# 412428728/ksched

Hardware: AMD Instinct MI355X
Metric: MCMF solve latency (ms) + arcs/s at 100k tasks x 10k machines, 1/2/4/8 GPUs (higher is better)
Workload: dtype int64; 1 GPU; config3: Quincy-shaped cell graph T=100000 M=10000 R=250 J=1000 (n=121252, m=531250), step = full device re-solve + device task->PU extraction (Solve() -> TaskMapping), one graph per GPU; tasks=100000, machines=10000, racks=250, jobs=1000, seed=3, n=121252, m=531250, parallelism=independent graphs x1

## Files before the change

include/ksmcmf.h:

```cpp
#ifndef KSMCMF_H
#define KSMCMF_H

#include <stddef.h>
#include <stdint.h>

#ifdef __cplusplus
extern "C" {
#endif

#define KSMCMF_ABI_VERSION 5

#define KS_OK            0
#define KS_E_INVALID    (-1)
#define KS_E_INFEASIBLE (-2)
#define KS_E_DEVICE     (-3)
#define KS_E_VERIFY     (-4)
#define KS_E_RANGE      (-5)

#define KS_NODE_OTHER    0
#define KS_NODE_TASK     1
#define KS_NODE_PU       2
#define KS_NODE_SINK     3
#define KS_NODE_MACHINE  4
#define KS_NODE_INTERMEDIATE 5
// ... 82 lines not shown
    uint64_t sweep_launches;
    double   ms_sweep_kernels;
    uint64_t gu_launches;
    double   ms_gu_kernels;
    int32_t  warm_started;
    int32_t  rebuilt;
    int32_t  recoveries;
    int32_t  solver;
    uint64_t fs_launches;
    double   ms_fs_kernels;
    uint64_t fwd_updates;
    int32_t  cells;
    int32_t  compact;
    double   ms_cell_kernel;
    uint64_t cell_ticks_max;
    uint64_t cell_ticks_sum;
    uint64_t fs_arc_scans;
    uint64_t cell_fallbacks;
    uint64_t cycles_cancelled;
    uint64_t fb_resets;
    uint64_t cycles_rejected;
    uint64_t gu_leaf_scans;
    int32_t  cells_run;
    int32_t  reserved4;
    uint64_t reserved3[1];
} ks_result;

typedef struct ks_store_stats {
    int64_t  live_arcs;
    int64_t  inserted;
    int64_t  updated;
    int64_t  killed;
    int64_t  superseded;
    int64_t  rebuilds;
    int64_t  residual_slots;
    int64_t  reserved[4];
} ks_store_stats;

typedef struct ks_flow {
    uint64_t src, dst;
    int64_t  flow;
} ks_flow;

int         ks_abi_version(void);
void        ks_default_opts(ks_opts* opts);
ks_ctx*     ks_create(int device, const ks_opts* opts);
void        ks_destroy(ks_ctx* ctx);
const char* ks_last_error(ks_ctx* ctx);
// ... 299 lines not shown
```

ksched_amd/csrc/ks_engine.hip:

```cpp
#include <hip/hip_runtime.h>

#include <algorithm>
#include <chrono>
#include <cstdio>
#include <cstdlib>
#include <cstring>
#include <vector>

#include "ks_engine_impl.h"
#include "ks_len.h"

namespace ks {
namespace {

__device__ __forceinline__ void seg_of(const long long* nd, int x, int& b0, int& b1) {
    const unsigned long long w = (unsigned long long)nd[ni(x) + ND_SEG];
    b0 = (int)(unsigned)(w & 0xffffffffULL);
    b1 = (int)(unsigned)(w >> 32);
}

__device__ __forceinline__ long long atom_add_ret(long long* p, long long v) {
    return __hip_atomic_fetch_add(p, v, __ATOMIC_RELAXED, __HIP_MEMORY_SCOPE_AGENT);
}
__device__ __forceinline__ long long atom_exch(long long* p, long long v) {
// ... 1074 lines not shown
                                         int& out, int& scans, int& lscan) {
    const int lig = lane_id() & (G - 1);
    long long dv = INF64;
    if (v >= 0) dv = atom_load(&g.dist[ni(v)]);
    const bool act = v >= 0 && (PR || dv < INF64);
    long long pv = 0;
    int b0 = 0, en = 0;
    if (act) {
        pv = g.p0[ni(v)];
        seg_of(g.p0, v, b0, en);
    }
    const int iters = G < 64 ? 1 : (en - b0 + 63) / 64;
    for (int it = 0; it < iters; ++it) {
        const int a = b0 + it * G + lig;
        if (a < en) {
            relax_in<PR, CP>(g, nf, Q, v, a, dkey<PR>(dv), pv, er, B, hub_min, out, lscan);
            scans++;
        }
    }
}

template <int PR, bool CP>
__global__ __launch_bounds__(BLK) void k_bf_round(DG g, int seq, int dense_arg) {
    const unsigned long long t_entry = PR == 2 ? __builtin_amdgcn_s_memrealtime() : 0;
    const int dense = __builtin_amdgcn_readfirstlane(dense_arg >= 0 ? dense_arg : (seq == g.ctl->bf_seq0 ? 1 : 0));
    __shared__ long long hub_min[HUB_LDS];
    __shared__ QEnt bfq[BF_DEPTH][BFQ_CAP];
    __shared__ int bfq_n[BF_DEPTH];
    if (blockIdx.x == 0) {
        for (int h = threadIdx.x; h < g.nheavy; h += BLK) g.bf[(seq + 2) % 3].hub[h] = 0;
        if (threadIdx.x == 0) g.ctl->bfa[(seq + 2) % 3] = 0;
    }
    const Front F = g.bf[seq % 3], N = g.bf[(seq + 1) % 3];
    if (threadIdx.x < HUB_LDS) hub_min[threadIdx.x] = INF64;
    if (threadIdx.x < BF_DEPTH) bfq_n[threadIdx.x] = 0;
    const int qcap = g.expand < 2 ? 0 : (g.expand == 2 ? BFQ_CAP : 2);
    const int qlo = qcap ? g.obeg[2] : 0, qhi = qcap ? g.obeg[CCLS] : 0;
    const BfQ Q{bfq[0], &bfq_n[0], qcap, qlo, qhi};
    __syncthreads();
    int done = 0, any = 0;
    auto ctl_words = [&]() {
        done = g.ctl->bf_done;
        any = g.ctl->bfa[seq % 3];
    };
    auto ctl_uniform = [&]() {
        done = __builtin_amdgcn_readfirstlane(done);
        any = __builtin_amdgcn_readfirstlane(any);
// ... 85 lines not shown
            const int qn = min(bfq_n[l], qcap);
            const BfQ Qn{bfq[l + 1 < BF_DEPTH ? l + 1 : 0], &bfq_n[l + 1 < BF_DEPTH ? l + 1 : 0],
                         l + 1 < BF_DEPTH ? qcap : 0, l + 1 < BF_DEPTH ? qlo : 0, l + 1 < BF_DEPTH ? qhi : 0};
            bf_drain<PR, CP>(g, N, bfq[l], qn, Qn, er, B, hub_min, out, scans, lscan);
            __syncthreads();
        }
    }
    if (threadIdx.x < HUB_LDS && (int)threadIdx.x < g.nheavy) {
        const long long val = hub_min[threadIdx.x];
        if (val < INF64) {
            long long* dx = &g.dist[ni(g.hub_base + threadIdx.x)];
            if (dless<PR>(val, atom_load(dx)) && dless<PR>(val, atom_min_ret(dx, val))) {
                N.hub[threadIdx.x] = 1;
                out = 1;
            }
        }
    }
    if (__any(out) && lane_id() == 0) g.ctl->bfa[(seq + 1) % 3] = 1;
    if (blockIdx.x == 0 && threadIdx.x == 0) {
        if (PR == 2 && g.ctl->t_srch) {
            g.ctl->srch_ticks += t_entry - g.ctl->t_srch;
            g.ctl->t_srch = 0;
        }
        if (!done && (dense || any)) {
            atomicAdd(g.ctr + C_BFROUND, 1ULL);
            g.ctl->bf_count += 1;
        } else if (!done) {
            g.ctl->bf_done = 1;
        }
    }
    if (!PR && g.bound && blockIdx.x == 0 && threadIdx.x < WAVE && !done && (dense || any)) {
        const int nb = g.ctl->n_bx;
        if (nb > 0 && nb <= BX_CAP) {
            long long d = 0;
            if ((int)threadIdx.x < nb) d = atom_load(&g.dist[ni(g.bx[threadIdx.x])]);
            d = wave_max(d);
            if (threadIdx.x == 0 && d < INF64)
                __hip_atomic_fetch_min(&g.ctl->bf_bound, d, __ATOMIC_RELAXED, __HIP_MEMORY_SCOPE_AGENT);
        }
    }
    scans = wave_sum(scans);
    lscan = wave_sum(lscan);
    if (lane_id() == 0 && (scans | lscan)) {
        const int sh = ((blockIdx.x * WPB) + (threadIdx.x >> 6)) & (CTR_SHARDS - 1);
        if (scans) atomicAdd(g.ctr + sh * NCTR + C_GUSCAN, (unsigned long long)scans);
        if (lscan) atomicAdd(g.ctr + sh * NCTR + C_GULEAF, (unsigned long long)lscan);
// ... 4 lines not shown
    for (long long i = blockIdx.x * (long long)BLK + threadIdx.x; i < g.hub_base; i += (long long)gridDim.x * BLK) {
        fs[0].flag[i] = 0;
        fs[1].flag[i] = 0;
        fs[2].flag[i] = 0;
    }
    if (blockIdx.x == 0)
        for (int h = threadIdx.x; h < g.nheavy; h += BLK) fs[0].hub[h] = fs[1].hub[h] = fs[2].hub[h] = 0;
}

__device__ __forceinline__ void bx_append(const DG& g, bool on, int v) {
    const unsigned long long m = __ballot(on);
    if (!m) return;
    int base = 0;
    if (lane_id() == 0) base = atomicAdd(&g.ctl->n_bx, (int)__popcll(m));
    base = __shfl(base, 0);
    if (on) {
        const int idx = base + (int)__popcll(m & ((1ULL << lane_id()) - 1));
        if (idx < BX_CAP) g.bx[idx] = v;
    }
}

__global__ void k_gu_init(DG g, int seq0, int list) {
    if (g.ctl->gu_pending) return;
    clear_fronts(g, g.bf);
    const Front F0 = g.bf[seq0 % 3];
    if (blockIdx.x == 0 && threadIdx.x == 0) {
        __hip_atomic_store(&g.ctl->bf_bound, INF64, __ATOMIC_RELAXED, __HIP_MEMORY_SCOPE_AGENT);
        g.ctl->gu_B = INF64;
        g.ctl->bf_done = 0;
        g.ctl->gu_L = 0;
        g.ctl->gu_X = -1;
        g.ctl->bf_r0 = g.ctl->bf_count;
        g.ctl->bf_seq0 = seq0;
        g.ctl->n_exc = 0;
        g.ctl->u_exc = 0;
        g.ctl->aug_reached = 0;
        g.ctl->aug_short = 0;
        for (int k = 0; k < 3; ++k) g.ctl->bfa[k] = k == seq0 % 3 ? 1 : 0;
    }
    for (long long v0 = blockIdx.x * (long long)BLK; v0 < g.hub_base; v0 += (long long)gridDim.x * BLK) {
        const long long v = v0 + threadIdx.x;
        long long e = 0;
        if (v < g.hub_base) {
            e = atom_load(&g.excess[v]);
            g.dist[ni(v)] = e < 0 ? 0 : INF64;
            if (e < 0) F0.flag[v] = 1;
// ... 5 lines not shown
            const int h = h0 + threadIdx.x;
            long long e = 0;
            if (h < g.nheavy) {
                drain_inbox(g, h);
                e = atom_load(&g.excess[g.hub_base + h]);
                g.dist[ni(g.hub_base + h)] = e < 0 ? 0 : INF64;
                if (e < 0) F0.hub[h] = 1;
            }
            if (list) bx_append(g, e > 0, g.hub_base + h);
        }
}

__global__ void k_pr_init(DG g, int seq0, int from_p) {
    clear_fronts(g, g.bf);
    if (blockIdx.x == 0 && threadIdx.x == 0) {
        g.ctl->bf_done = 0;
        g.ctl->bf_seq0 = seq0;
        for (int k = 0; k < 3; ++k) g.ctl->bfa[k] = 0;
    }
    for (long long v = blockIdx.x * (long long)BLK + threadIdx.x; v < g.n; v += (long long)gridDim.x * BLK)
        g.dist[ni(v)] = from_p == 2 ? ((PK_BIAS << PK_NB) | PK_NONE) : from_p ? g.p0[ni(v)] : 0;
}

__global__ void k_cycle_end(DG g, Ctl* host, int fwd) {
    static_assert(sizeof(Ctl) % 4 == 0, "Ctl is copied as words");
    const unsigned long long t = __builtin_amdgcn_s_memrealtime();
    if (threadIdx.x == 0) {
        if (!fwd) g.ctl->gu_pending = g.ctl->bf_done ? 0 : 1;
        g.ctl->t_end = t;
    }
    __syncthreads();
    const int* src = reinterpret_cast<const int*>(g.ctl);
    int* dst = reinterpret_cast<int*>(host);
    for (int i = threadIdx.x; i < (int)(sizeof(Ctl) / 4); i += blockDim.x)
        __hip_atomic_store(&dst[i], src[i], __ATOMIC_RELAXED, __HIP_MEMORY_SCOPE_SYSTEM);
    __syncthreads();
    if (threadIdx.x == 0) {
        if (!fwd) {
            g.ctl->n_exc = 0;
            g.ctl->u_exc = 0;
        }
        g.ctl->fs_moved_cyc = 0;
    }
    __threadfence_system();
}

constexpr int SET_FWD = 1;
constexpr int SET_CYC = 2;
__global__ void k_set_eps(DG g, long long eps, double inv, int flags) {
    g.ctl->eps = eps;
    g.ctl->inv = inv;
    g.ctl->lim = (1LL << 60) / eps;
// ... 3 lines not shown
        g.ctl->fs_completed = 0;
    }
    if (flags & SET_CYC) {
        g.ctl->cyc_done = 0;
        g.ctl->cyc_rej = 0;
    }
}

__global__ void k_prc_snap(DG g, Ctl* host) {
    const unsigned long long t = __builtin_amdgcn_s_memrealtime();
    if (threadIdx.x == 0 && g.ctl->t_srch) {
        g.ctl->srch_ticks += t - g.ctl->t_srch;
        g.ctl->t_srch = 0;
    }
    __syncthreads();
    const int* src = reinterpret_cast<const int*>(g.ctl);
    int* dst = reinterpret_cast<int*>(host);
    for (int i = threadIdx.x; i < (int)(sizeof(Ctl) / 4); i += blockDim.x)
        __hip_atomic_store(&dst[i], src[i], __ATOMIC_RELAXED, __HIP_MEMORY_SCOPE_SYSTEM);
    __threadfence_system();
}

__global__ void k_gu_max(DG g) {
    __shared__ long long sh[WPB];
    clear_fronts(g, g.sf);
    if (blockIdx.x == 0) {
        for (int k = threadIdx.x; k < MAXB; k += BLK) g.ctl->sweep_act[k] = 0;
        for (int h = threadIdx.x; h < g.nheavy; h += BLK) {
            g.aug_req[h] = 0;
        }
        if (threadIdx.x == 0) {
            g.ctl->apply_act = 0;
            g.ctl->n_xl2 = 0;
        }
    }
    if (!g.ctl->bf_done) return;
    if (g.bound && blockIdx.x == 0 && threadIdx.x < WAVE) {
        const int nb = g.ctl->n_bx;
        if (nb > 0 && nb <= BX_CAP) {
            long long d = 0;
            if ((int)threadIdx.x < nb) d = atom_load(&g.dist[ni(g.bx[threadIdx.x])]);
            d = wave_max(d);
            if (threadIdx.x == 0) g.ctl->gu_B = d;
        }
        if (threadIdx.x == 0) g.ctl->n_bx = 0;
    }
    long long mx = 0;
    long long mxx = -1;
    for (long long v = blockIdx.x * (long long)BLK + threadIdx.x; v < g.n; v += (long long)gridDim.x * BLK) {
        const long long d = atom_load(&g.dist[ni(v)]);
        if (d < INF64) mx = max(mx, d);
        if (d < INF64 && atom_load(&g.excess[v]) > 0) mxx = max(mxx, d);
    }
    mx = wave_max(mx);
    const int w = threadIdx.x >> 6;
    if (lane_id() == 0) sh[w] = mx;
// ... 1017 lines not shown
int Engine::device() const { return p_->device; }

int Engine::init(int device, const ks_opts& opts, std::string& err) {
    EngineImpl& s = *p_;
    s.device = device;
    s.opts = opts;
    int ndev = 0;
    KS_CHECK(hipGetDeviceCount(&ndev));
    if (device < 0 || device >= ndev) {
        err = "device index out of range";
        return KS_E_DEVICE;
    }
    KS_CHECK(hipSetDevice(device));
    KS_CHECK(hipStreamCreateWithFlags(&s.stream, hipStreamNonBlocking));
    {
        int v = 0;
        if (hipDeviceGetAttribute(&v, hipDeviceAttributeSharedMemPerBlockOptin, device) != hipSuccess || v <= 0)
            KS_CHECK(hipDeviceGetAttribute(&v, hipDeviceAttributeMaxSharedMemoryPerBlock, device));
        s.lds_limit = (size_t)std::max(v, 0);
    }
    for (auto& e : s.ev) KS_CHECK(hipEventCreate(&e));
    for (auto& e : s.kev) KS_CHECK(hipEventCreate(&e));
    for (auto& e : s.fin_ev) KS_CHECK(hipEventCreate(&e));
    for (auto& c : s.cev)
        for (auto& e : c) KS_CHECK(hipEventCreate(&e));
    for (auto& c : s.fev)
        for (auto& e : c) KS_CHECK(hipEventCreate(&e));
    for (auto& e : s.cdone) KS_CHECK(hipEventCreate(&e));
    for (int i = 0; i < CYC_SLOTS; ++i) {
        KS_CHECK(hipHostMalloc(&s.h_cyc[i], sizeof(Ctl), hipHostMallocCoherent | hipHostMallocMapped));
        std::memset(s.h_cyc[i], 0, sizeof(Ctl));
        KS_CHECK(hipHostGetDevicePointer((void**)&s.d_cyc[i], s.h_cyc[i], 0));
    }
    KS_CHECK(s.ctl.ensure(1));
    KS_CHECK(s.ctr.ensure(CTR_SHARDS * NCTR));
    KS_CHECK(s.xl.ensure(AUG_KMAX));
    KS_CHECK(s.xl2.ensure(AUG_K2));
    KS_CHECK(s.bx.ensure(BX_CAP));
    KS_CHECK(s.fdef.ensure(FDEF_CAP));
    KS_CHECK(s.sctl.ensure(1));
    KS_CHECK(hipMemset(s.sctl.p, 0, sizeof(StoreCtl)));
    KS_CHECK(hipHostMalloc(&s.h_ctl, sizeof(Ctl)));
    KS_CHECK(hipHostMalloc(&s.h_sctl, sizeof(StoreCtl)));
    std::memset(s.h_sctl, 0, sizeof(StoreCtl));
    return KS_OK;
}

void Engine::set_cells(const int64_t* off, size_t k) {
// ... 66 lines not shown
    EngineImpl& s;
    ks_result& res;
    std::string& err;
    const ks_opts& o;
    const hipStream_t st;
    const std::chrono::steady_clock::time_point t_host0 = std::chrono::steady_clock::now();
    const bool fb;
    const bool use_warm;
    Retry retry = RETRY_NONE;
    bool run_all = true;
    std::vector<int> run_list;
    int cells_run = 0;

    int hi = 0, nn = 0, ncells = 0;
    int64_t m2 = 0;
    long long mult = 1, maxc = 0;
    bool cpv = false;
    DG g{};

    int alpha = 8, gi_base = 24, gi_tail = 4, pr_cap = 160, prc_cap = 4096, kb_margin = 6, kb_min = 8;
    long long pr_div = 32;
    int phase_exit = 256, phase_frac = 128, aug_slack = 4, walk_passes = 1, fwd_k = 64;
    bool use_pr = false, use_prc = false, use_fwd = false, use_aug = false, cycle_log = false;
    int cyc_lg = CYC_LOG;
    int nhit = 0;
    int fgrid = 0, dgrid = 0, sgrid = 0, wgrid = 0, ngrid = 0, fsgrid = 0, vgrid = 0;
    long long eps_start = 1;

    uint64_t sweeps = 0, gus = 0, sweep_launches = 0, bf_launches = 0, sweep_kernels = 0, early_exits = 0;
    uint64_t fwd_updates = 0, fs_launches = 0;
    double ms_bf_k = 0, ms_sw_k = 0, ms_fs_k = 0;
    double ms_sat = 0, ms_cycles = 0, ms_pr = 0, ms_cell = 0;
    int phases = 0;
    int prc_cycles = 0, prc_searches = 0;
    long long prc_rejected = 0;
    unsigned long long cell_ctr[5] = {0, 0, 0, 0, 0};
    unsigned long long cell_rounds = 0, cticks_max = 0, cticks_sum = 0;
    long long tot_cost = 0, tot_flow = 0;
    bool launch_refused = false;
    bool cost_range = false, cost_wide = false;
    double cost_mag = 0;
    unsigned long long gu_prev = 0;

    long long eps = 1;
    int kb = 24;
    int kf = 16;
    int sseq = 0, bseq = 0;
    bool cp_dirty = false;
    int status = KS_OK;
    bool pr_failed = false;
    bool prc_tried = false;
    long long solve_units = -1;
    long long warm_thr = 0;

    struct Phase {
        long long eps = 1;
        int wsl = 1;
        bool early = false;
        int* prc_early = nullptr;
        uint64_t sweeps = 0;
        int gi = 0;
        int peak = 0;
        int list = 0;
        int fwd = 0;
        int fwd_block = 0;
        int fwd_budget = 64;
        bool first_upd = true;
        int nupd = 1;
        int completed0 = 0;
        int cur = 0;
        int bf_pend = -1;
        int rc = KS_OK;
    } ph;

    struct Finish {
        int2 *JMa, *JMb;
        int *J0, *onc, *R, *gbad;
        int* indeg;
        long long *gsum, *gcap;
        bool lds_search;
        int nsearch, cap, used;
        int nb;
        unsigned long long srch_seen;
    } fin{};

    SolveRun(EngineImpl& s_, ks_result& res_, std::string& err_, bool warm)
        : s(s_), res(res_), err(err_), o(s_.opts), st(s_.stream), fb(s_.fb_active),
          use_warm((warm && s_.has_prev) || s_.fb_active) {}

    double wall_s() const {
        return std::chrono::duration<double>(std::chrono::steady_clock::now() - t_host0).count();
    }

    int run() {
// ... 157 lines not shown
        g.fs_wide = std::max(2048, nn / 4);
        g.aug_k = o.tail_nodes > 0 ? std::min(AUG_KMAX, (int)o.tail_nodes) : 64;
        fgrid = s.window_grid();
        dgrid = s.dense_grid();
        sgrid = s.sparse_grid();
        wgrid = s.sweep_grid();
        ngrid = grid_for(nn, 2048);
        fsgrid = s.nhitems * HSPLIT + FS_LIST_BLOCKS;
        vgrid = grid_for(hi, VERIFY_GRID);
        use_fwd = o.fwd_nodes >= 0 && s.m2cap < FS_NONE;
        fwd_k = o.fwd_nodes > 0 ? (int)o.fwd_nodes : (nn < 32768 ? 32 : 64);
        use_pr = o.price_refine != 0;
        use_prc = use_pr && o.price_refine == 1 && !s.cell_layout && s.m2cap < PK_NONE;
        alpha = o.alpha >= 2 ? o.alpha : (!s.cell_layout && nn < 32768 && use_prc) ? 32 : 8;
        gi_base = o.gu_interval > 0 ? o.gu_interval : 24;
        gi_base = std::max(2, std::min(MAXB, gi_base)) & ~1;
        pr_cap = o.pr_rounds > 0 ? o.pr_rounds : 160;
        cycle_log = o.log_cycles != 0;
        nhit = s.nhitems;
        use_aug = o.walk_slack >= 0;
        aug_slack = o.walk_slack > 0 ? o.walk_slack : 4;
        walk_passes = o.walk_passes > 0 ? std::min(8, (int)o.walk_passes) : 1;
        kb_margin = o.bf_margin > 0 ? o.bf_margin : 6;
        kb_min = 8;
        prc_cap = (o.fault_inject & 32) ? 32 : 4096;
        cyc_lg = (o.fault_inject & 128) ? 5 : CYC_LOG;
        gi_tail = o.tail_sweeps > 0 ? std::max(2, std::min(MAXB, (int)o.tail_sweeps)) & ~1 : 4;
        phase_exit = o.phase_exit < 0 ? 0 : (o.phase_exit > 0 ? o.phase_exit : 256);
        phase_frac = o.phase_frac > 0 ? o.phase_frac : 128;
        eps = std::max<long long>(1, maxc * mult);
        {
            const long long D = o.final_div < 0 ? 0
                                : o.final_div > 0 ? o.final_div
                                : (s.cell_layout || nn < 32768) ? 20 : (use_prc ? 24 : 48);
            if (D > 0 && use_pr && maxc > 0) {
                long long e = std::max<long long>(1, (mult - 1) / D);
                if (s.cell_layout && (alpha & (alpha - 1)) == 0)
                    while (e & (e - 1)) e &= e - 1;
                const long long lo = std::max<long long>(1, eps / ((long long)alpha * alpha));
                while (e < lo && e <= (1LL << 58) / alpha) e *= alpha;
                eps = e * alpha;
                pr_div = D;
            }
        }
        eps_start = eps;
    }

// ... 111 lines not shown
                else pr_failed = true;
            }
        } while (eps > 1);
        return KS_OK;
    }

    int run_phase(long long eps_ph, long long sat_thr, bool may_end_early, int walk_sl, int* prc_early = nullptr) {
        KS_CHECK(hipEventRecord(s.ev[2], st));
        KS_CHECK(set_eps(eps_ph, use_fwd ? SET_FWD : 0));
        KS_HOT(cpv, k_saturate, fgrid, BLK, st, g, sat_thr);
        cp_dirty = cpv;
        KS_CHECK(hipEventRecord(s.ev[3], st));
        ph = Phase{};
        ph.eps = eps_ph;
        ph.wsl = walk_sl;
        ph.early = may_end_early;
        ph.prc_early = prc_early;
        ph.gi = gi_base;
        for (;;) {
            const int r = ph.fwd ? fwd_cycle() : bwd_cycle();
            if (r < 0) return r;
            if (r == PHASE_OVER) break;
        }
        flush_bf();
        KS_CHECK(hipEventRecord(s.ev[4], st));
        KS_CHECK(hipEventSynchronize(s.ev[4]));
        ms_sat += ev_ms(s.ev[2], s.ev[3]);
        ms_cycles += ev_ms(s.ev[3], s.ev[4]);
        return ph.rc;
    }

    hipError_t enqueue_fwd(int par, int nupd) {
        hipError_t e = hipSuccess;
        for (int u = 0; u < nupd; ++u) {
            hipLaunchKernelGGL(k_fs_init, dim3(ngrid), dim3(BLK), 0, st, g, bseq);
            if ((e = hipEventRecord(s.fev[par][2 * u], st)) != hipSuccess) return e;
            for (int r = 0; r < kf; ++r) {
                KS_HOT(cpv, k_fs_round, fsgrid, BLK, st, g, bseq);
                ++bseq;
                ++fs_launches;
            }
            if ((e = hipEventRecord(s.fev[par][2 * u + 1], st)) != hipSuccess) return e;
            hipLaunchKernelGGL(k_fs_apply, dim3(ngrid), dim3(BLK), 0, st, g);
            KS_HOT(cpv, k_fs_trace, FDEF_CAP, WAVE, st, g);
            hipLaunchKernelGGL(k_fs_end, dim3(1), dim3(WAVE), 0, st, g);
        }
        hipLaunchKernelGGL(k_cycle_end, dim3(1), dim3(128), 0, st, g, s.d_cyc[par], 1);
        return hipEventRecord(s.cdone[par], st);
    }
    int fwd_cycle() {
        KS_CHECK(enqueue_fwd(ph.cur, ph.nupd));
        KS_CHECK(hipEventSynchronize(s.cdone[ph.cur]));
        const Ctl* hc = s.h_cyc[ph.cur];
        double t_fs = 0;
        for (int u = 0; u < ph.nupd; ++u) t_fs += ev_ms(s.fev[ph.cur][2 * u], s.fev[ph.cur][2 * u + 1]);
        ms_fs_k += t_fs;
        ph.cur ^= 1;
        const bool completed = hc->fs_done || hc->fs_fail;
        if (cycle_log)
            std::fprintf(stderr, "fwd cycle phase %d eps %lld updates %d rounds %d fs_ms %.3f units %lld n_exc %d done %d fail %d D %lld deficits %d moved %d width %d\n",
                         phases, ph.eps, ph.nupd, hc->fs_rounds, t_fs, hc->u_exc_rep, hc->n_exc_rep,
                         hc->fs_done, hc->fs_fail, hc->fs_D < FS_DMAX ? hc->fs_D : -1LL, hc->n_fdef,
                         hc->fs_moved_cyc, hc->fs_maxcnt);
        if (completed && hc->n_exc_rep == 0) return PHASE_OVER;
        const int done_now = hc->fs_completed - ph.completed0;
        ph.completed0 = hc->fs_completed;
        gus += done_now;
        fwd_updates += done_now;
        bool wide = hc->fs_fail == 2;
        if (!completed && hc->fs_rounds >= ph.fwd_budget) {
            KS_CHECK(hipMemsetAsync(&s.ctl.p->fs_pending, 0, sizeof(int), st));
            KS_CHECK(hipMemsetAsync(s.ctl.p->fs_cnt, 0, sizeof(s.ctl.p->fs_cnt), st));
            wide = true;
        }
        if (hc->fs_fail || wide) {
            ph.fwd = 0;
            ph.fwd_block = 1;
            ph.nupd = 1;
            return CYCLE_NEXT;
        }
        if (!completed) {
            kf = std::min(256, 2 * kf);
            ph.nupd = 1;
            return CYCLE_NEXT;
        }
        kf = std::max(8, std::min(256, hc->fs_rounds + 4));
        ph.nupd = FWD_UPD;
        if (hc->fs_moved_cyc == 0) {
            ph.fwd = 0;
            ph.fwd_block = 1;
        }
        if (wall_s() > kSolveWallLimitS) {
            (void)hipStreamSynchronize(st);
            err = "forward tail did not converge (" + std::to_string(wall_s()) + " s)";
            return KS_E_DEVICE;
        }
        return CYCLE_NEXT;
    }

    hipError_t enqueue_bwd(int par) {
        const int gi = ph.gi, wsl = ph.wsl;
        hipLaunchKernelGGL(k_gu_init, dim3(ngrid), dim3(BLK), 0, st, g, bseq, ph.list);
        hipError_t e = hipEventRecord(s.cev[par][0], st);
        if (e != hipSuccess) return e;
        for (int r = 0; r < kb; ++r) bf_round(0, false);
        if ((e = hipEventRecord(s.cev[par][1], st)) != hipSuccess) return e;
        hipLaunchKernelGGL(k_gu_max, dim3(ngrid), dim3(BLK), 0, st, g);
        hipLaunchKernelGGL(k_gu_apply, dim3(ngrid), dim3(BLK), 0, st, g, sseq);
        if (use_aug) {
            KS_HOT(cpv, k_augment, g.aug_k, WAVE, st, g, sseq, 0, wsl);
            if (nhit) KS_HOT(cpv, k_aug_hub, nhit, BLK, st, g, sseq, wsl);
            KS_HOT(cpv, k_augment, AUG_K2, WAVE, st, g, sseq, 1, wsl);
            for (int wp = 1; wp < walk_passes; ++wp)
                KS_HOT(cpv, k_augment, g.aug_k, WAVE, st, g, sseq, 0, wsl);
        }
        for (int k = 0; k < gi; ++k) KS_HOT(cpv, k_sweep, wgrid, BLK, st, g, k, sseq + k);
        hipLaunchKernelGGL(k_cycle_end, dim3(1), dim3(128), 0, st, g, s.d_cyc[par], 0);
        sseq += gi;
        return hipEventRecord(s.cdone[par], st);
    }
    void flush_bf() {
        if (ph.bf_pend >= 0) ms_bf_k += ev_ms(s.cev[ph.bf_pend][0], s.cev[ph.bf_pend][1]);
        ph.bf_pend = -1;
    }
    int bwd_cycle() {
        const int cur = ph.cur, gi = ph.gi;
        if (ph.bf_pend == cur) flush_bf();
        KS_CHECK(enqueue_bwd(cur));
        flush_bf();
        KS_CHECK(hipEventSynchronize(s.cdone[cur]));
        const Ctl* hc = s.h_cyc[cur];
        sweep_kernels += gi;
        double t_bf = 0;
        if (cycle_log) {
            t_bf = ev_ms(s.cev[cur][0], s.cev[cur][1]);
            ms_bf_k += t_bf;
        } else {
            ph.bf_pend = cur;
        }
        const double t_sw = hc->t_end > hc->t_sw0 ? (double)(hc->t_end - hc->t_sw0) / 1e5 : 0.0;
        ms_sw_k += t_sw;
        if (hc->infeasible) {
            ph.rc = KS_E_INFEASIBLE;
            std::memcpy(s.h_ctl, hc, sizeof(Ctl));
            return PHASE_OVER;
        }
        if (!hc->bf_done) {
            kb = std::min(256, kb * 2);
            ph.cur ^= 1;
            return CYCLE_NEXT;
        }
        if (cycle_log) {
            unsigned long long relax = 0;
            if (int rc = relaxations(&relax)) return rc;
            std::fprintf(stderr, "cycle phase %d eps %lld bf %d relax %llu bf_ms %.3f sw_ms %.3f active %d units %lld n_exc %d walks %d/%d",
                         phases, ph.eps, hc->bf_count - hc->bf_r0, relax, t_bf, t_sw, hc->sweep_act[gi - 1], hc->u_exc, hc->n_exc,
                         hc->aug_reached, hc->aug_short);
            for (int k = 0; k < std::min(4, hc->n_exc); ++k) {
                const int x = hc->dbg_x[k];
                int c = 0;
                while (c < NGC && x >= s.obeg[c + 1]) ++c;
                std::fprintf(stderr, " [x%d c%d e%d]", x, x >= s.hub_base ? 9 : c, hc->dbg_e[k]);
            }
            std::fprintf(stderr, "\n");
        }
        if (ph.first_upd) {
            ph.first_upd = false;
            if (solve_units < 0) solve_units = hc->u_exc;
            if (ph.prc_early && ph.early && hc->u_exc * kPrcUnitsDiv <= solve_units) {
                ph.early = false;
                *ph.prc_early = 1;
            }
        }
        kb = std::max(kb_min, std::min(256, hc->bf_count - hc->bf_r0 + kb_margin));
        ph.fwd_budget = std::max(16, 2 * (hc->bf_count - hc->bf_r0));
        ++gus;
        sweeps += gi;
        sweep_launches += gi;
        ph.sweeps += gi;
        int last = 0;
        for (int k = 0; k < gi; ++k)
            if (hc->sweep_act[k]) last = k + 1;
        if (!hc->sweep_act[gi - 1]) {
            sweeps -= gi - last;
            return PHASE_OVER;
        }
        ph.peak = std::max(ph.peak, hc->n_exc);
        if (ph.early && hc->n_exc <= phase_exit && (long long)hc->n_exc * phase_frac <= ph.peak) {
            ++early_exits;
            return PHASE_OVER;
        }

        ph.gi = (use_aug && hc->n_exc <= g.aug_k) ? gi_tail : gi_base;
        ph.list = g.bound && hc->n_exc > 0 && hc->n_exc <= BX_CAP;
        ph.fwd = use_fwd && ph.early && !ph.fwd_block && hc->n_exc > 0 && hc->n_exc <= fwd_k;
        ph.fwd_block = 0;
        if (ph.sweeps > (uint64_t)(64 * ((uint64_t)nn + 64)) || wall_s() > kSolveWallLimitS) {
            (void)hipStreamSynchronize(st);
            err = "push/relabel did not converge (sweeps " + std::to_string(ph.sweeps) + ", " +
                  std::to_string(wall_s()) + " s)";
            return KS_E_DEVICE;
        }
        ph.cur ^= 1;
        return CYCLE_NEXT;
    }

    int price_refine(long long eps_try, int* rounds_used, int cap, int from_p = 0) {
        KS_CHECK(hipEventRecord(s.ev[5], st));
        KS_CHECK(set_eps(eps_try));
        hipLaunchKernelGGL(k_pr_init, dim3(ngrid), dim3(BLK), 0, st, g, bseq, from_p);
        int used = 0, ok = 0;
        for (int batch = 0; used < cap; ++batch) {
            const int k = std::min(64, cap - used);
            KS_CHECK(hipEventRecord(s.kev[0], st));
            bf_rounds(1, k, batch == 0);
            KS_CHECK(hipEventRecord(s.kev[1], st));
            used += k;
            KS_CHECK(read_ctl());
// ... 438 lines not shown
        res.ms_phase[2] = ms_cycles;
        res.ms_phase[3] = ms_pr;
        res.ms_phase[4] = ev_ms(s.ev[5], s.ev[6]);
        res.ms_phase[5] = 1e3 * wall_s();
        res.gu_arc_scans = tc[C_GUSCAN];
        res.gu_leaf_scans = tc[C_GULEAF];
        res.fs_arc_scans = tc[C_FSSCAN];
        res.sweep_launches = sweep_kernels;
        res.ms_sweep_kernels = ms_sw_k;
        res.gu_launches = bf_launches;
        res.ms_gu_kernels = ms_bf_k;
        res.fs_launches = fs_launches;
        res.ms_fs_kernels = ms_fs_k;
        res.fwd_updates = fwd_updates;
        res.solver = s.cell_layout ? 1 : 0;
        res.cells = s.cell_layout ? ncells : 0;
        res.cells_run = s.cell_layout ? cells_run : 0;
        res.ms_cell_kernel = ms_cell;
        res.cell_ticks_max = cticks_max;
        res.cell_ticks_sum = cticks_sum;
        res.status = status;
        res.cycles_cancelled = (uint64_t)prc_cycles;
        res.cycles_rejected = (uint64_t)prc_rejected;
        KS_CHECK(hipMemsetAsync(s.n_cshift.p, 0, s.nstore * sizeof(unsigned long long), st));
        if (status == KS_OK) {
            KS_CHECK(hipMemsetAsync(s.n_fresh.p, 0, s.nstore, st));
            if (s.cell_first_valid && s.cell_dirty.p)
                KS_CHECK(hipMemsetAsync(s.cell_dirty.p, 0, (s.cell_off.size() - 1) * sizeof(int), st));
            KS_CHECK(hipStreamSynchronize(st));
            s.solved = true;
            s.has_prev = true;
            s.cells_kept = s.cell_layout;
        } else {
            s.has_prev = false;
            s.cells_kept = false;
        }
        return status;
    }
};

}

int Engine::solve(ks_result& res, bool warm, std::string& err) {
    EngineImpl& s = *p_;
    KS_CHECK(hipSetDevice(s.device));
    SolveRun run(s, res, err, warm);
// ... 31 lines not shown
```

ksched_amd/csrc/ks_engine_impl.h:

```cpp
#pragma once

#include <hip/hip_runtime.h>

#include <algorithm>
#include <cstdint>
#include <string>
#include <vector>

#include "ks_cell.h"
#include "ks_engine.h"
#include "ks_sched.h"

namespace ks {
namespace impl {

constexpr int BLK = 256;
constexpr int WAVE = 64;
constexpr int WPB = BLK / WAVE;
constexpr int NGC = 6;
constexpr int HEAVY_MIN = 4096;
constexpr int CHUNK = 1024;
constexpr int PER_T = CHUNK / 256;
constexpr int HSPLIT = 4;
constexpr int BF_PER_T = PER_T / HSPLIT;
// ... 49 lines not shown
    int dbg_x[4];
    int dbg_e[4];
    int n_bx;
    long long bf_bound;
    long long gu_B;
    long long fs_D;
    int fs_cnt[3];
    int fs_done;
    int fs_fail;
    int fs_pending;
    int fs_rounds;
    int n_fdef;
    int fs_moved;
    long long u_exc;
    int fs_maxcnt;
    int n_exc_rep;
    long long u_exc_rep;
    int fs_completed;
    int fs_moved_cyc;
    unsigned long long t_sw0;
    unsigned long long t_end;
    unsigned long long t_srch;
    unsigned long long srch_ticks;
    long long lim;
};

struct HItem {
    int node, hid, begin, end;
};

__host__ __device__ constexpr int class_lanes(int c) { return c < 4 ? (4 << c) : 64; }
__host__ __device__ inline int degree_class(int d) {
    return d <= 4 ? 0 : d <= 8 ? 1 : d <= 16 ? 2 : d <= 32 ? 3 : d <= 64 ? 4 : d <= HEAVY_MIN ? 5 : NGC;
}
constexpr int CCLS = 5;

struct CItem {
    int node, begin, end, lead;
};
__host__ __device__ constexpr int win_batches(int c) { return c < 4 ? 2 : 1; }
static_assert(NGC == 6, "KS_BY_CLASS dispatches six classes");
__host__ __device__ constexpr int win_slots(int c) { return win_batches(c) * (64 / class_lanes(c)); }

struct Front {
    unsigned char* flag;
    int* hub;
};

// ... 87 lines not shown
        if (e == hipSuccess) e = hipStreamSynchronize(st);
        if (p) (void)hipFree(p);
        p = q;
        n = want;
        return e;
    }
    void release() {
        if (p) (void)hipFree(p);
        p = nullptr;
        n = 0;
    }
};

}
using namespace impl;

struct EngineImpl {
    int device = 0;
    ks_opts opts{};
    hipStream_t stream = nullptr;
    hipEvent_t ev[7] = {};
    hipEvent_t kev[4] = {};
    hipEvent_t fin_ev[4] = {};
    hipEvent_t cev[CYC_SLOTS][2] = {};
    hipEvent_t fev[CYC_SLOTS][8] = {};
    hipEvent_t cdone[CYC_SLOTS] = {};
    Ctl* h_cyc[CYC_SLOTS] = {};
    Ctl* d_cyc[CYC_SLOTS] = {};

    int64_t nstore = 0;
    int64_t nslots = 0;
    DBuf<long long> n_supply;
    DBuf<unsigned char> n_type, n_alive, n_fresh;
    DBuf<unsigned long long> n_cshift;
    DBuf<int> n_lastrm;
    DBuf<int> n_hint;
    DBuf<unsigned char> n_grow;
    DBuf<unsigned long long> n_bind;
    int64_t acap = 0;
    DBuf<int> a_src, a_dst, fwd, free_stack;
    DBuf<long long> a_low, a_cap, a_cost;
    DBuf<unsigned char> a_alive, a_type;
    int64_t hcap = 0;
    DBuf<unsigned long long> hkey;
    DBuf<int> hval, hlast;
    DBuf<StoreCtl> sctl;
    StoreCtl* h_sctl = nullptr;
// ... 100 lines not shown
        d.a_src = a_src.p;
        d.a_dst = a_dst.p;
        d.a_low = a_low.p;
        d.a_cap = a_cap.p;
        d.a_cost = a_cost.p;
        d.fwd = fwd.p;
        d.first = first.p;
        d.used = used.p;
        d.pos = pos.p;
        d.ent = ent.p;
        d.mult = mult;
        d.csr_valid = csr_valid ? 1 : 0;
        return d;
    }

    ~EngineImpl() {
        if (stream) {
            (void)hipSetDevice(device);
            (void)hipStreamSynchronize(stream);
        }
        if (h_ctl) (void)hipHostFree(h_ctl);
        for (auto* h : h_cyc)
            if (h) (void)hipHostFree(h);
        for (auto& c : cev)
            for (auto& e : c)
                if (e) (void)hipEventDestroy(e);
        for (auto& c : fev)
            for (auto& e : c)
                if (e) (void)hipEventDestroy(e);
        for (auto& e : cdone)
            if (e) (void)hipEventDestroy(e);
        if (h_sctl) (void)hipHostFree(h_sctl);
        for (auto& e : ev)
            if (e) (void)hipEventDestroy(e);
        for (auto& e : kev)
            if (e) (void)hipEventDestroy(e);
        for (auto& e : fin_ev)
            if (e) (void)hipEventDestroy(e);
        if (stream) (void)hipStreamDestroy(stream);
    }

    StoreDev sd() const {
        StoreDev d{};
        d.ncap = (int)ncap;
        d.n_supply = n_supply.p;
        d.n_type = n_type.p;
        d.n_alive = n_alive.p;
        d.n_fresh = n_fresh.p;
        d.n_cshift = n_cshift.p;
// ... 126 lines not shown
```

ksched_amd/native.py:

```python
from __future__ import annotations

import ctypes as C
import os
from dataclasses import dataclass

import numpy as np

from . import _build

KS_OK, KS_E_INVALID, KS_E_INFEASIBLE, KS_E_DEVICE, KS_E_VERIFY, KS_E_RANGE = 0, -1, -2, -3, -4, -5
KS_ADD_NODE, KS_REMOVE_NODE, KS_ADD_ARC, KS_UPDATE_ARC, KS_SET_EXCESS = 0, 1, 2, 3, 4

EXPORTED_SYMBOLS = (
    "ks_abi_version", "ks_default_opts", "ks_create", "ks_destroy", "ks_last_error", "ks_load_graph",
    "ks_apply_deltas", "ks_solve", "ks_get_flows", "ks_get_task_mapping", "ks_get_task_pu_device", "ks_solve_many",
    "ks_coalesce_deltas", "ks_get_store_stats", "ks_set_bindings", "ks_scheduling_deltas",
    "ks_update_unsched_costs", "ks_topology_stats", "ks_get_graph", "ks_commit_schedule",
    "ks_commit_preemptive", "ks_remove_resources", "ks_complete_tasks", "ks_get_bindings",
    "ks_add_tasks", "ks_add_resources", "ks_update_tasks", "ks_update_nodes",
    "ks_batch_create", "ks_batch_create_rank", "ks_batch_unique_id", "ks_batch_destroy", "ks_batch_last_error",
    "ks_batch_load", "ks_batch_solve", "ks_batch_gather",
    "ks_batch_slots", "ks_batch_owner", "ks_batch_block_len", "ks_batch_unpack",
    "ks_batch_node_offsets", "ks_batch_translate_deltas", "ks_batch_reserve", "ks_batch_apply_deltas",
    "ks_batch_get_graph", "ks_batch_set_bindings", "ks_batch_commit_schedule", "ks_batch_commit_preemptive",
# ... 34 lines not shown
                ("phase_exit", C.c_int32), ("phase_frac", C.c_int32), ("tail_sweeps", C.c_int32),
                ("bf_margin", C.c_int32), ("two_hop", C.c_int32), ("log_cycles", C.c_int32),
                ("fault_inject", C.c_int32), ("walk_passes", C.c_int32), ("tail_nodes", C.c_int32),
                ("bf_bound", C.c_int32), ("fwd_nodes", C.c_int32), ("cell_nodes", C.c_int32),
                ("warm_shift", C.c_int32),
                ("warm_canon", C.c_int32),
                ("compact_pos", C.c_int32)]


class KsResult(C.Structure):
    _fields_ = [("total_cost", C.c_int64), ("flow_value", C.c_int64), ("status", C.c_int32),
                ("phases", C.c_int32), ("sweeps", C.c_uint64), ("arc_scans", C.c_uint64),
                ("node_visits", C.c_uint64), ("pushes", C.c_uint64), ("relabels", C.c_uint64),
                ("global_updates", C.c_uint64), ("gu_iterations", C.c_uint64), ("gu_arc_scans", C.c_uint64),
                ("ms_phase", C.c_double * 6), ("n_nodes", C.c_int64), ("n_arcs", C.c_int64),
                ("sweep_launches", C.c_uint64), ("ms_sweep_kernels", C.c_double),
                ("gu_launches", C.c_uint64), ("ms_gu_kernels", C.c_double), ("warm_started", C.c_int32),
                ("rebuilt", C.c_int32), ("recoveries", C.c_int32), ("solver", C.c_int32),
                ("fs_launches", C.c_uint64), ("ms_fs_kernels", C.c_double), ("fwd_updates", C.c_uint64),
                ("cells", C.c_int32), ("compact", C.c_int32), ("ms_cell_kernel", C.c_double),
                ("cell_ticks_max", C.c_uint64), ("cell_ticks_sum", C.c_uint64), ("fs_arc_scans", C.c_uint64),
                ("cell_fallbacks", C.c_uint64), ("cycles_cancelled", C.c_uint64), ("fb_resets", C.c_uint64),
                ("cycles_rejected", C.c_uint64), ("gu_leaf_scans", C.c_uint64), ("cells_run", C.c_int32),
                ("reserved4", C.c_int32), ("reserved3", C.c_uint64 * 1)]

    def as_dict(self) -> dict:
        d = {k: getattr(self, k) for k, _ in self._fields_ if k not in ("ms_phase", "reserved3", "reserved4")}
        names = ("build", "saturate", "cycles", "price_refine", "verify", "total")
        d["ms"] = dict(zip(names, list(self.ms_phase)))
        return d


class KsStoreStats(C.Structure):
    _fields_ = [("live_arcs", C.c_int64), ("inserted", C.c_int64), ("updated", C.c_int64),
                ("killed", C.c_int64), ("superseded", C.c_int64), ("rebuilds", C.c_int64),
                ("residual_slots", C.c_int64), ("reserved", C.c_int64 * 4)]

    def as_dict(self) -> dict:
        return {k: getattr(self, k) for k, _ in self._fields_ if k != "reserved"}


class KsCommitStats(C.Structure):
    _fields_ = [("placed", C.c_int64), ("arcs_removed", C.c_int64), ("running_added", C.c_int64),
                ("running_converted", C.c_int64), ("unsched_updates", C.c_int64), ("cap_updates", C.c_int64),
                ("records", C.c_int64), ("reserved", C.c_int64 * 5)]

    def as_dict(self) -> dict:
        return {k: getattr(self, k) for k, _ in self._fields_ if k != "reserved"}


# ... 801 lines not shown
```

Before: 16.89 million arcs/s.

## Speculatively enqueue next backward-cycle head before host reads cycle result

After each backward cycle, the host now enqueues the next cycle's init kernel and the first few Bellman-Ford rounds right away. Those head kernels gate themselves on a device-side decision (head_go, head_list), which mirrors the host's cycle_next rule, so the GPU keeps working while the host syncs and decides. Per-cycle BF timing moves from host events to device timestamps, which removes the event pair around the BF rounds. The change adds a host/device consistency check that fails hard on a mismatch, and it risks wasted or dropped head work.

Result: faster. 17.16 million arcs/s, median of 5 (+1.6%).

```diff
diff --git a/include/ksmcmf.h b/include/ksmcmf.h
--- a/include/ksmcmf.h
+++ b/include/ksmcmf.h
@@ -128,8 +128,8 @@
     uint64_t cycles_rejected;
     uint64_t gu_leaf_scans;
     int32_t  cells_run;
-    int32_t  reserved4;
-    uint64_t reserved3[1];
+    int32_t  cycle_heads;
+    uint64_t cycle_heads_dropped;
 } ks_result;
 
 typedef struct ks_store_stats {
diff --git a/ksched_amd/csrc/ks_engine.hip b/ksched_amd/csrc/ks_engine.hip
--- a/ksched_amd/csrc/ks_engine.hip
+++ b/ksched_amd/csrc/ks_engine.hip
@@ -1120,7 +1120,7 @@
 
 template <int PR, bool CP>
 __global__ __launch_bounds__(BLK) void k_bf_round(DG g, int seq, int dense_arg) {
-    const unsigned long long t_entry = PR == 2 ? __builtin_amdgcn_s_memrealtime() : 0;
+    const unsigned long long t_entry = PR != 1 ? __builtin_amdgcn_s_memrealtime() : 0;
     const int dense = __builtin_amdgcn_readfirstlane(dense_arg >= 0 ? dense_arg : (seq == g.ctl->bf_seq0 ? 1 : 0));
     __shared__ long long hub_min[HUB_LDS];
     __shared__ QEnt bfq[BF_DEPTH][BFQ_CAP];
@@ -1252,6 +1252,7 @@
             g.ctl->srch_ticks += t_entry - g.ctl->t_srch;
             g.ctl->t_srch = 0;
         }
+        if (PR == 0 && !done && !g.ctl->t_bf0) g.ctl->t_bf0 = t_entry;
         if (!done && (dense || any)) {
             atomicAdd(g.ctr + C_BFROUND, 1ULL);
             g.ctl->bf_count += 1;
@@ -1302,6 +1303,10 @@
 
 __global__ void k_gu_init(DG g, int seq0, int list) {
     if (g.ctl->gu_pending) return;
+    if (list < 0) {
+        if (!g.ctl->head_go) return;
+        list = g.ctl->head_list;
+    }
     clear_fronts(g, g.bf);
     const Front F0 = g.bf[seq0 % 3];
     if (blockIdx.x == 0 && threadIdx.x == 0) {
@@ -1353,12 +1358,15 @@
         g.dist[ni(v)] = from_p == 2 ? ((PK_BIAS << PK_NB) | PK_NONE) : from_p ? g.p0[ni(v)] : 0;
 }
 
-__global__ void k_cycle_end(DG g, Ctl* host, int fwd) {
+__global__ void k_cycle_end(DG g, Ctl* host, int fwd, CycleRule r) {
     static_assert(sizeof(Ctl) % 4 == 0, "Ctl is copied as words");
     const unsigned long long t = __builtin_amdgcn_s_memrealtime();
     if (threadIdx.x == 0) {
         if (!fwd) g.ctl->gu_pending = g.ctl->bf_done ? 0 : 1;
         g.ctl->t_end = t;
+        const int n_exc = g.ctl->n_exc;
+        g.ctl->head_go = !fwd && cycle_head_runs(cycle_next(*g.ctl, r)) ? 1 : 0;
+        g.ctl->head_list = g.bound && n_exc > 0 && n_exc <= BX_CAP ? 1 : 0;
     }
     __syncthreads();
     const int* src = reinterpret_cast<const int*>(g.ctl);
@@ -1408,6 +1416,7 @@
 }
 
 __global__ void k_gu_max(DG g) {
+    const unsigned long long t_entry = __builtin_amdgcn_s_memrealtime();
     __shared__ long long sh[WPB];
     clear_fronts(g, g.sf);
     if (blockIdx.x == 0) {
@@ -1418,6 +1427,10 @@
         if (threadIdx.x == 0) {
             g.ctl->apply_act = 0;
             g.ctl->n_xl2 = 0;
+            if (g.ctl->t_bf0) {
+                g.ctl->bf_ticks += t_entry - g.ctl->t_bf0;
+                g.ctl->t_bf0 = 0;
+            }
         }
     }
     if (!g.ctl->bf_done) return;
@@ -2481,8 +2494,6 @@
     for (auto& e : s.ev) KS_CHECK(hipEventCreate(&e));
     for (auto& e : s.kev) KS_CHECK(hipEventCreate(&e));
     for (auto& e : s.fin_ev) KS_CHECK(hipEventCreate(&e));
-    for (auto& c : s.cev)
-        for (auto& e : c) KS_CHECK(hipEventCreate(&e));
     for (auto& c : s.fev)
         for (auto& e : c) KS_CHECK(hipEventCreate(&e));
     for (auto& e : s.cdone) KS_CHECK(hipEventCreate(&e));
@@ -2595,6 +2606,8 @@
     long long pr_div = 32;
     int phase_exit = 256, phase_frac = 128, aug_slack = 4, walk_passes = 1, fwd_k = 64;
     bool use_pr = false, use_prc = false, use_fwd = false, use_aug = false, cycle_log = false;
+    bool no_head = false;
+    bool pin_kb = false;
     int cyc_lg = CYC_LOG;
     int nhit = 0;
     int fgrid = 0, dgrid = 0, sgrid = 0, wgrid = 0, ngrid = 0, fsgrid = 0, vgrid = 0;
@@ -2602,7 +2615,9 @@
 
     uint64_t sweeps = 0, gus = 0, sweep_launches = 0, bf_launches = 0, sweep_kernels = 0, early_exits = 0;
     uint64_t fwd_updates = 0, fs_launches = 0;
+    uint64_t heads = 0, heads_dropped = 0;
     double ms_bf_k = 0, ms_sw_k = 0, ms_fs_k = 0;
+    unsigned long long bf_seen = 0;
     double ms_sat = 0, ms_cycles = 0, ms_pr = 0, ms_cell = 0;
     int phases = 0;
     int prc_cycles = 0, prc_searches = 0;
@@ -2642,7 +2657,9 @@
         int nupd = 1;
         int completed0 = 0;
         int cur = 0;
-        int bf_pend = -1;
+        bool head = false;
+        CycleRule rule{};
+        bool rule_final = false;
         int rc = KS_OK;
     } ph;
 
@@ -2846,7 +2863,10 @@
         aug_slack = o.walk_slack > 0 ? o.walk_slack : 4;
         walk_passes = o.walk_passes > 0 ? std::min(8, (int)o.walk_passes) : 1;
         kb_margin = o.bf_margin > 0 ? o.bf_margin : 6;
-        kb_min = 8;
+        kb_min = HEAD_ROUNDS;
+        no_head = (o.fault_inject & 1024) != 0;
+        pin_kb = (o.fault_inject & 2048) != 0;
+        if (pin_kb) kb = kb_min;
         prc_cap = (o.fault_inject & 32) ? 32 : 4096;
         cyc_lg = (o.fault_inject & 128) ? 5 : CYC_LOG;
         gi_tail = o.tail_sweeps > 0 ? std::max(2, std::min(MAXB, (int)o.tail_sweeps)) & ~1 : 4;
@@ -3004,7 +3024,6 @@
             if (r < 0) return r;
             if (r == PHASE_OVER) break;
         }
-        flush_bf();
         KS_CHECK(hipEventRecord(s.ev[4], st));
         KS_CHECK(hipEventSynchronize(s.ev[4]));
         ms_sat += ev_ms(s.ev[2], s.ev[3]);
@@ -3027,7 +3046,7 @@
             KS_HOT(cpv, k_fs_trace, FDEF_CAP, WAVE, st, g);
             hipLaunchKernelGGL(k_fs_end, dim3(1), dim3(WAVE), 0, st, g);
         }
-        hipLaunchKernelGGL(k_cycle_end, dim3(1), dim3(128), 0, st, g, s.d_cyc[par], 1);
+        hipLaunchKernelGGL(k_cycle_end, dim3(1), dim3(128), 0, st, g, s.d_cyc[par], 1, CycleRule{});
         return hipEventRecord(s.cdone[par], st);
     }
     int fwd_cycle() {
@@ -3038,6 +3057,11 @@
         for (int u = 0; u < ph.nupd; ++u) t_fs += ev_ms(s.fev[ph.cur][2 * u], s.fev[ph.cur][2 * u + 1]);
         ms_fs_k += t_fs;
         ph.cur ^= 1;
+        if (!hc->bf_done) {
+            (void)hipStreamSynchronize(st);
+            err = "a dropped cycle head ran: the backward update before a forward cycle is no longer converged";
+            return KS_E_DEVICE;
+        }
         const bool completed = hc->fs_done || hc->fs_fail;
         if (cycle_log)
             std::fprintf(stderr, "fwd cycle phase %d eps %lld updates %d rounds %d fs_ms %.3f units %lld n_exc %d done %d fail %d D %lld deficits %d moved %d width %d\n",
@@ -3082,11 +3106,10 @@
 
     hipError_t enqueue_bwd(int par) {
         const int gi = ph.gi, wsl = ph.wsl;
-        hipLaunchKernelGGL(k_gu_init, dim3(ngrid), dim3(BLK), 0, st, g, bseq, ph.list);
-        hipError_t e = hipEventRecord(s.cev[par][0], st);
-        if (e != hipSuccess) return e;
-        for (int r = 0; r < kb; ++r) bf_round(0, false);
-        if ((e = hipEventRecord(s.cev[par][1], st)) != hipSuccess) return e;
+        int rounds = kb;
+        if (ph.head) rounds = std::max(0, kb - HEAD_ROUNDS);
+        else hipLaunchKernelGGL(k_gu_init, dim3(ngrid), dim3(BLK), 0, st, g, bseq, ph.list);
+        for (int r = 0; r < rounds; ++r) bf_round(0, false);
         hipLaunchKernelGGL(k_gu_max, dim3(ngrid), dim3(BLK), 0, st, g);
         hipLaunchKernelGGL(k_gu_apply, dim3(ngrid), dim3(BLK), 0, st, g, sseq);
         if (use_aug) {
@@ -3097,38 +3120,65 @@
                 KS_HOT(cpv, k_augment, g.aug_k, WAVE, st, g, sseq, 0, wsl);
         }
         for (int k = 0; k < gi; ++k) KS_HOT(cpv, k_sweep, wgrid, BLK, st, g, k, sseq + k);
-        hipLaunchKernelGGL(k_cycle_end, dim3(1), dim3(128), 0, st, g, s.d_cyc[par], 0);
+        ph.rule = CycleRule{gi, ph.early ? 1 : 0, ph.peak, phase_exit, phase_frac,
+                            use_fwd && !ph.fwd_block ? 1 : 0, fwd_k};
+        ph.rule_final = !ph.first_upd;
+        hipLaunchKernelGGL(k_cycle_end, dim3(1), dim3(128), 0, st, g, s.d_cyc[par], 0, ph.rule);
         sseq += gi;
-        return hipEventRecord(s.cdone[par], st);
-    }
-    void flush_bf() {
-        if (ph.bf_pend >= 0) ms_bf_k += ev_ms(s.cev[ph.bf_pend][0], s.cev[ph.bf_pend][1]);
-        ph.bf_pend = -1;
+        const hipError_t e = hipEventRecord(s.cdone[par], st);
+        if (e != hipSuccess) return e;
+        ph.head = ph.rule_final && !no_head;
+        if (ph.head) {
+            hipLaunchKernelGGL(k_gu_init, dim3(ngrid), dim3(BLK), 0, st, g, bseq, -1);
+            for (int r = 0; r < HEAD_ROUNDS; ++r) bf_round(0, false);
+        }
+        return hipSuccess;
     }
     int bwd_cycle() {
         const int cur = ph.cur, gi = ph.gi;
-        if (ph.bf_pend == cur) flush_bf();
         KS_CHECK(enqueue_bwd(cur));
-        flush_bf();
+        const Ctl* hc = s.h_cyc[cur];
         KS_CHECK(hipEventSynchronize(s.cdone[cur]));
-        const Ctl* hc = s.h_cyc[cur];
         sweep_kernels += gi;
-        double t_bf = 0;
-        if (cycle_log) {
-            t_bf = ev_ms(s.cev[cur][0], s.cev[cur][1]);
-            ms_bf_k += t_bf;
-        } else {
-            ph.bf_pend = cur;
-        }
+        const double t_bf = (double)(hc->bf_ticks - bf_seen) / 1e5;
+        bf_seen = hc->bf_ticks;
+        ms_bf_k += t_bf;
         const double t_sw = hc->t_end > hc->t_sw0 ? (double)(hc->t_end - hc->t_sw0) / 1e5 : 0.0;
         ms_sw_k += t_sw;
-        if (hc->infeasible) {
+        CycleRule rule = ph.rule;
+        if (ph.first_upd && !hc->infeasible && hc->bf_done) {
+            ph.first_upd = false;
+            if (solve_units < 0) solve_units = hc->u_exc;
+            if (ph.prc_early && ph.early && hc->u_exc * kPrcUnitsDiv <= solve_units) {
+                ph.early = false;
+                *ph.prc_early = 1;
+            }
+            rule.early = ph.early ? 1 : 0;
+        }
+        const int next = cycle_next(*hc, rule);
+        const int list = g.bound && hc->n_exc > 0 && hc->n_exc <= BX_CAP;
+        if (ph.rule_final) {
+            const int go = cycle_head_runs(next) ? 1 : 0;
+            if (hc->head_go != go || (next == CYC_BWD && hc->head_list != list)) {
+                (void)hipStreamSynchronize(st);
+                err = "the device's and the host's decision after a cycle differ (host " + std::to_string(next) +
+                      " list " + std::to_string(list) + ", device head_go " + std::to_string(hc->head_go) +
+                      " head_list " + std::to_string(hc->head_list) + ")";
+                return KS_E_DEVICE;
+            }
+        }
+        if (ph.head) {
+            if (cycle_head_runs(next)) ++heads;
+            else ++heads_dropped;
+            ph.head = cycle_head_runs(next);
+        }
+        if (next == CYC_INFEASIBLE) {
             ph.rc = KS_E_INFEASIBLE;
             std::memcpy(s.h_ctl, hc, sizeof(Ctl));
             return PHASE_OVER;
         }
-        if (!hc->bf_done) {
-            kb = std::min(256, kb * 2);
+        if (next == CYC_PENDING) {
+            if (!pin_kb) kb = std::min(256, kb * 2);
             ph.cur ^= 1;
             return CYCLE_NEXT;
         }
@@ -3146,36 +3196,28 @@
             }
             std::fprintf(stderr, "\n");
         }
-        if (ph.first_upd) {
-            ph.first_upd = false;
-            if (solve_units < 0) solve_units = hc->u_exc;
-            if (ph.prc_early && ph.early && hc->u_exc * kPrcUnitsDiv <= solve_units) {
-                ph.early = false;
-                *ph.prc_early = 1;
-            }
-        }
-        kb = std::max(kb_min, std::min(256, hc->bf_count - hc->bf_r0 + kb_margin));
+        if (!pin_kb) kb = std::max(kb_min, std::min(256, hc->bf_count - hc->bf_r0 + kb_margin));
         ph.fwd_budget = std::max(16, 2 * (hc->bf_count - hc->bf_r0));
         ++gus;
         sweeps += gi;
         sweep_launches += gi;
         ph.sweeps += gi;
-        int last = 0;
-        for (int k = 0; k < gi; ++k)
-            if (hc->sweep_act[k]) last = k + 1;
-        if (!hc->sweep_act[gi - 1]) {
+        if (next == CYC_DRAINED) {
+            int last = 0;
+            for (int k = 0; k < gi; ++k)
+                if (hc->sweep_act[k]) last = k + 1;
             sweeps -= gi - last;
             return PHASE_OVER;
         }
         ph.peak = std::max(ph.peak, hc->n_exc);
-        if (ph.early && hc->n_exc <= phase_exit && (long long)hc->n_exc * phase_frac <= ph.peak) {
+        if (next == CYC_EARLY) {
             ++early_exits;
             return PHASE_OVER;
         }
 
         ph.gi = (use_aug && hc->n_exc <= g.aug_k) ? gi_tail : gi_base;
-        ph.list = g.bound && hc->n_exc > 0 && hc->n_exc <= BX_CAP;
-        ph.fwd = use_fwd && ph.early && !ph.fwd_block && hc->n_exc > 0 && hc->n_exc <= fwd_k;
+        ph.list = list;
+        ph.fwd = next == CYC_FWD;
         ph.fwd_block = 0;
         if (ph.sweeps > (uint64_t)(64 * ((uint64_t)nn + 64)) || wall_s() > kSolveWallLimitS) {
             (void)hipStreamSynchronize(st);
@@ -3660,6 +3702,8 @@
         res.status = status;
         res.cycles_cancelled = (uint64_t)prc_cycles;
         res.cycles_rejected = (uint64_t)prc_rejected;
+        res.cycle_heads = (int32_t)heads;
+        res.cycle_heads_dropped = heads_dropped;
         KS_CHECK(hipMemsetAsync(s.n_cshift.p, 0, s.nstore * sizeof(unsigned long long), st));
         if (status == KS_OK) {
             KS_CHECK(hipMemsetAsync(s.n_fresh.p, 0, s.nstore, st));
diff --git a/ksched_amd/csrc/ks_engine_impl.h b/ksched_amd/csrc/ks_engine_impl.h
--- a/ksched_amd/csrc/ks_engine_impl.h
+++ b/ksched_amd/csrc/ks_engine_impl.h
@@ -95,8 +95,33 @@
     unsigned long long t_end;
     unsigned long long t_srch;
     unsigned long long srch_ticks;
+    unsigned long long t_bf0;
+    unsigned long long bf_ticks;
     long long lim;
-};
+    int head_go;
+    int head_list;
+};
+
+enum CycleNext { CYC_PENDING = 0, CYC_BWD, CYC_FWD, CYC_DRAINED, CYC_EARLY, CYC_INFEASIBLE };
+struct CycleRule {
+    int gi;
+    int early;
+    int peak;
+    int phase_exit, phase_frac;
+    int fwd_ok;
+    int fwd_k;
+};
+__host__ __device__ inline int cycle_next(const Ctl& c, const CycleRule& r) {
+    if (c.infeasible) return CYC_INFEASIBLE;
+    if (!c.bf_done) return CYC_PENDING;
+    if (!c.sweep_act[r.gi - 1]) return CYC_DRAINED;
+    const int peak = r.peak > c.n_exc ? r.peak : c.n_exc;
+    if (r.early && c.n_exc <= r.phase_exit && (long long)c.n_exc * r.phase_frac <= peak) return CYC_EARLY;
+    if (r.fwd_ok && r.early && c.n_exc > 0 && c.n_exc <= r.fwd_k) return CYC_FWD;
+    return CYC_BWD;
+}
+__host__ __device__ inline bool cycle_head_runs(int next) { return next == CYC_PENDING || next == CYC_BWD; }
+constexpr int HEAD_ROUNDS = 8;
 
 struct HItem {
     int node, hid, begin, end;
@@ -230,7 +255,6 @@
     hipEvent_t ev[7] = {};
     hipEvent_t kev[4] = {};
     hipEvent_t fin_ev[4] = {};
-    hipEvent_t cev[CYC_SLOTS][2] = {};
     hipEvent_t fev[CYC_SLOTS][8] = {};
     hipEvent_t cdone[CYC_SLOTS] = {};
     Ctl* h_cyc[CYC_SLOTS] = {};
@@ -377,9 +401,6 @@
         if (h_ctl) (void)hipHostFree(h_ctl);
         for (auto* h : h_cyc)
             if (h) (void)hipHostFree(h);
-        for (auto& c : cev)
-            for (auto& e : c)
-                if (e) (void)hipEventDestroy(e);
         for (auto& c : fev)
             for (auto& e : c)
                 if (e) (void)hipEventDestroy(e);
diff --git a/ksched_amd/native.py b/ksched_amd/native.py
--- a/ksched_amd/native.py
+++ b/ksched_amd/native.py
@@ -80,10 +80,10 @@
                 ("cell_ticks_max", C.c_uint64), ("cell_ticks_sum", C.c_uint64), ("fs_arc_scans", C.c_uint64),
                 ("cell_fallbacks", C.c_uint64), ("cycles_cancelled", C.c_uint64), ("fb_resets", C.c_uint64),
                 ("cycles_rejected", C.c_uint64), ("gu_leaf_scans", C.c_uint64), ("cells_run", C.c_int32),
-                ("reserved4", C.c_int32), ("reserved3", C.c_uint64 * 1)]
+                ("cycle_heads", C.c_int32), ("cycle_heads_dropped", C.c_uint64)]
 
     def as_dict(self) -> dict:
-        d = {k: getattr(self, k) for k, _ in self._fields_ if k not in ("ms_phase", "reserved3", "reserved4")}
+        d = {k: getattr(self, k) for k, _ in self._fields_ if k != "ms_phase"}
         names = ("build", "saturate", "cycles", "price_refine", "verify", "total")
         d["ms"] = dict(zip(names, list(self.ms_phase)))
         return d
```
